# labgem/pangenomeNEM

Measured on AMD Instinct MI355X. Metric: em_family_x_organism_cells_per_sec, higher is better.
Workload: dtype f32 chains with f64 intermediates (reference arithmetic); int32 popcounts in the M-step; 1 GPU; BASELINE configs[1]: 20000 families x 500 organisms, K=3, beta=0.5, contiguity graph (path + 5% chords, weights 1..8), ncem/sk_/pk; U-shaped family-frequency spectrum (Beta(0.3, 0.3) per family), default .m init; families_total=20000, families_per_gpu=20000, organisms=500, K=3, parallelism=1 GPU

## Files before the change

### pangenomenem_amd/csrc/nem_kernels.hip

```cpp
#include <hip/hip_runtime.h>
#include <cstdlib>
#include <algorithm>
#include <cfloat>
#include <cstdint>
#include <cstring>
#include <type_traits>

#include "nem_ff.hpp"
#include "nem_chain.hpp"
#include "nem_halfsum.hpp"
#include "nem_kernels.hpp"
#include "nem_sweep_dev.hpp"

namespace nemk {

#ifdef NEM_PHASE_PROF
__device__ unsigned long long g_phase[32];
#define NEM_PHASE(i) do { if (blockIdx.x == 0 && threadIdx.x == 0) g_phase[i] = wall_clock64(); } while (0)
#else
#define NEM_PHASE(i) do { } while (0)
#endif


__device__ __forceinline__ int stat_sum(const int* __restrict__ stats, int idx, int ranks, int stride)
{
    int s = stats[idx];
    for (int r = 1; r < ranks; r++) s += stats[idx + r * stride];
    return s;
}

__device__ inline int wave_reduce_add(int v)
{
    v += __builtin_amdgcn_update_dpp(0, v, 0xB1, 0xF, 0xF, false);
    v += __builtin_amdgcn_update_dpp(0, v, 0x4E, 0xF, 0xF, false);
    v += __builtin_amdgcn_update_dpp(0, v, 0x141, 0xF, 0xF, false);
    v += __builtin_amdgcn_update_dpp(0, v, 0x140, 0xF, 0xF, false);
    v += __builtin_amdgcn_update_dpp(0, v, 0x142, 0xA, 0xF, false);
    v += __builtin_amdgcn_update_dpp(0, v, 0x143, 0xC, 0xF, false);
    return __builtin_amdgcn_readlane(v, 63);
}

__device__ inline long long wave_reduce_add_ll(long long v)
{
    const int lo = wave_reduce_add((int)(v & 0xFFFFF));
    const int hi = wave_reduce_add((int)(v >> 20));
    return ((long long)hi << 20) + (long long)lo;
}

__device__ __forceinline__ float chain_add16(float s, const float4& a, const float4& b, const float4& c, const float4& d)
{
    asm volatile("v_add_f32 %0, %0, %1\n\tv_add_f32 %0, %0, %2\n\tv_add_f32 %0, %0, %3\n\tv_add_f32 %0, %0, %4\n\t"
                 "v_add_f32 %0, %0, %5\n\tv_add_f32 %0, %0, %6\n\tv_add_f32 %0, %0, %7\n\tv_add_f32 %0, %0, %8\n\t"
                 "v_add_f32 %0, %0, %9\n\tv_add_f32 %0, %0, %10\n\tv_add_f32 %0, %0, %11\n\tv_add_f32 %0, %0, %12\n\t"
// ... 99 lines not shown
    }
}

constexpr int DCH = 512;

__device__ __forceinline__ bool density_tile(int K, int ntiles, int& tile, int& k)
{
    const int b = blockIdx.x;
    const int g = b / (8 * K), r = b - g * (8 * K);
    k = r >> 3;
    tile = g * 8 + (r & 7);
    return tile < ntiles;
}

__device__ __forceinline__ float bern_step(float dk, uint32_t m, int b, double l1h, double l0)
{
    const uint32_t hi = ((b <= 30) ? (m << (30 - b)) : (m >> 1)) & 0x40000000u;
    const double f = __hiloint2double((int)hi, 0);
    return (float)(fma(f, l1h, (double)dk) - l0);
}

__device__ __forceinline__ uint32_t word_of(const uint4& v, int c)
{
    return c == 0 ? v.x : c == 1 ? v.y : c == 2 ? v.z : v.w;
}

__device__ __forceinline__ uint32_t mismatch_word(uint32_t x, const uint2 am)
{
    uint32_t m;
    asm("v_bfi_b32 %0, %1, %2, %3" : "=v"(m) : "v"(x), "v"(am.y), "v"(am.x));
    return m;
}

__device__ __forceinline__ float chain_plain(const uint4* __restrict__ xw4, int npad, int i, int D,
                                    const uint2* am, double l1h, double l0)
{
    float dk = 0.0f;
    const int wlast = (D - 1) >> 5;
    const int glast = wlast >> 2;
    uint4 xn = xw4[i];
    for (int g = 0; g <= glast; g++) {
        const uint4 xv = xn;
        if (g < glast) xn = xw4[(size_t)(g + 1) * npad + i];
#pragma unroll
        for (int c = 0; c < 4; c++) {
            const int w = 4 * g + c;
            if (w > wlast) break;
            const uint32_t m = mismatch_word(word_of(xv, c), am[w]);
            const int nb = (w < wlast) ? 32 : (D - (wlast << 5));
            if (nb == 32) {
#pragma unroll
                for (int b = 0; b < 32; b++) dk = bern_step(dk, m, b, l1h, l0);
            } else {
                for (int b = 0; b < nb; b++) dk = bern_step(dk, m, b, l1h, l0);
            }
        }
    }
    return dk;
}

constexpr int kFFPlainWords = 1;
#ifndef NEM_FF_PLAIN_STEPS
#define NEM_FF_PLAIN_STEPS 32
#endif
constexpr int kFFPlainSteps = NEM_FF_PLAIN_STEPS;

__device__ __forceinline__ void ff_load(const uint32_t* sQ0, const uint32_t* sDQ, uint32_t bits, uint32_t& q0, uint32_t& dq,
                                        uint32_t& end)
{
    const uint32_t E = (bits >> 23) & 255u;
    q0 = sQ0[E];
    dq = sDQ[E];
    end = (E + 1u) << 23;
// ... 48 lines not shown
            bits = ff_probe(mm, j, dq, at);
            bits = ff_exact_step(bits, mm, j, l1h, l0);
            ff_load(sQ0, sDQ, bits, q0, dq, end);
            rem -= (int)j + 1;
            if (rem <= 0) break;
            mm = mm >> (j + 1u);
            const uint32_t c2 = ff_cand(mm, dq, mad24((uint32_t)rem, q0, bits));
            if (c2 < end) { bits = c2; break; }
        }
    }
}

__device__ __forceinline__ void ff_group(const uint4& xv, int g, const uint2* am, uint32_t& bits,
                                         uint32_t& q0, uint32_t& q1, uint32_t& end, const uint32_t* sQ0,
                                         const uint32_t* sQ1, double l1h, double l0)
{
#pragma unroll
    for (int c = 0; c < 4; c++) {
        const int w = 4 * g + c;
        const uint32_t m = mismatch_word(word_of(xv, c), am[w]);
        if (c < kFFPlainWords && g == 0) {
            float dk0 = __uint_as_float(bits);
#pragma unroll
            for (int b = 0; b < kFFPlainSteps; b++) dk0 = bern_step(dk0, m, b, l1h, l0);
            bits = __float_as_uint(dk0);
            ff_load(sQ0, sQ1, bits, q0, q1, end);
            if (kFFPlainSteps < 32) ff_word(bits, q0, q1, end, m >> kFFPlainSteps, 32 - kFFPlainSteps, sQ0, sQ1, l1h, l0);
        } else {
            ff_word(bits, q0, q1, end, m, 32, sQ0, sQ1, l1h, l0);
        }
    }
}

__device__ __forceinline__ float chain_ff(const uint4* __restrict__ xw4, int npad, int i, int D,
                                          const uint2* am, const uint32_t* sQ0,
                                          const uint32_t* sQ1, double l1h, double l0)
{
    const int wlast = (D - 1) >> 5;
    const int gfull = wlast >> 2;
    uint32_t bits = 0u;
    uint32_t q0, q1, end;
    ff_load(sQ0, sQ1, bits, q0, q1, end);
    const uint4* pn = xw4 + i;
    int gi = 0;
    auto next = [&]() {
        const uint4 v = *pn;
        if (gi < gfull) { pn += npad; gi++; }
        return v;
    };
    uint4 x0 = next(), x1 = next(), x2 = next(), x3 = next();
    int g = 0;
    for (; g + 4 <= gfull; g += 4) {
        ff_group(x0, g, am, bits, q0, q1, end, sQ0, sQ1, l1h, l0);
        x0 = next();
        ff_group(x1, g + 1, am, bits, q0, q1, end, sQ0, sQ1, l1h, l0);
        x1 = next();
        ff_group(x2, g + 2, am, bits, q0, q1, end, sQ0, sQ1, l1h, l0);
        x2 = next();
        ff_group(x3, g + 3, am, bits, q0, q1, end, sQ0, sQ1, l1h, l0);
        x3 = next();
    }
    uint4 xt = x0;
    if (g < gfull) { ff_group(x0, g, am, bits, q0, q1, end, sQ0, sQ1, l1h, l0); xt = x1; g++; }
    if (g < gfull) { ff_group(x1, g, am, bits, q0, q1, end, sQ0, sQ1, l1h, l0); xt = x2; g++; }
    if (g < gfull) { ff_group(x2, g, am, bits, q0, q1, end, sQ0, sQ1, l1h, l0); xt = x3; g++; }
#pragma unroll
    for (int c = 0; c < 4; c++) {
        const int w = 4 * gfull + c;
        if (w > wlast) break;
        uint32_t m = mismatch_word(word_of(xt, c), am[w]);
        const int nb = (w < wlast) ? 32 : (D - (wlast << 5));
        if (nb < 32) m &= (1u << nb) - 1u;
        ff_word(bits, q0, q1, end, m, nb, sQ0, sQ1, l1h, l0);
    }
    return __uint_as_float(bits);
}

__device__ __forceinline__ void ff_build(uint32_t* sQ0, uint32_t* sDQ, double l1, double l0, int tid)
{
    uint32_t q0, q1;
    ff_entry(l1, -l0, tid, q0, q1);
    if (q0 == kFFInvalid) q1 = kFFInvalid;
    sQ0[tid] = q0; sDQ[tid] = q1 - q0;
}

__device__ __forceinline__ void density_store(const int* __restrict__ perm, int tile, int tid, int n, int npad, int k,
                                              float dk, uint32_t nul, double pk, float logpk,
                                              double* __restrict__ pkfki, float* __restrict__ logpkfki)
{
    __shared__ double sPk[256];
    __shared__ float sLp[256];
    float logfk; double fk;
    if (!nul) { logfk = -dk; fk = exp((double)logfk); }
    else { logfk = -FLT_MAX; fk = 0.0; }
    const int slot = perm[tile * 256 + tid] - tile * 256;
    sPk[slot] = pk * fk;
    sLp[slot] = logpk + logfk;
    __syncthreads();
    const int io = tile * 256 + tid;
    if (io < n) {
        pkfki[(size_t)k * npad + io] = sPk[tid];
        logpkfki[(size_t)k * npad + io] = sLp[tid];
    }
}

struct DensityArgs {
    const uint4* xw; int n, npad, dpad, D, K;
    const double2* tabT; const double* tabL0; const uint32_t* nz0; const uint32_t* nz1;
    const uint32_t* am0; const uint32_t* am1; const double2* uni; const int* nonuni;
    const double* pk; const float* logpk;
    double* pkfki; float* logpkfki;
    int* zero_flags; int n_zero_flags;
    const int* stop;
    int use_ff;
    const int* perm;
    const uint2* ffq;
};

__device__ __forceinline__ void density_body(const DensityArgs& a)
{
    __shared__ double2 sT[DCH];
    __shared__ double sL[DCH];
    __shared__ uint32_t sQ0[256], sQ1[256];
    __shared__ uint2 sAm[kDensMaskWords];
    if (a.stop != nullptr && *a.stop) return;
    int k, tile;
    if (!density_tile(a.K, a.npad >> 8, tile, k)) return;
    const int tid = threadIdx.x;
    const int i = tile * 256 + tid;
    const int npad = a.npad, dpad = a.dpad;
    const int W = dpad >> 5;
    float dk = 0.0f;
    uint32_t nul = 0;
    if (tile == 0 && k == 0)
        for (int t = tid; t < a.n_zero_flags; t += 256) a.zero_flags[t] = 0;

    if (a.nonuni[k] == 0) {
        const double l1 = a.uni[k].x, l0 = a.uni[k].y;
        const double l1h = 0.5 * l1;
        for (int w = tid; w < W; w += 256) sAm[w] = make_uint2(a.am0[k * W + w], a.am1[k * W + w]);
        if (a.use_ff && l1 >= 0.0 && l0 <= 0.0) {
            const uint2 q = a.ffq[k * 256 + tid];
            sQ0[tid] = q.x; sQ1[tid] = q.y;
            __syncthreads();
            dk = chain_ff(a.xw, npad, i, a.D, sAm, sQ0, sQ1, l1h, l0);
        } else {
            __syncthreads();
            dk = chain_plain(a.xw, npad, i, a.D, sAm, l1h, l0);
        }
    } else {
        for (int d0 = 0; d0 < dpad; d0 += DCH) {
            const int dn = min(DCH, dpad - d0);
            __syncthreads();
            for (int t = tid; t < dn; t += 256) {
                sT[t] = a.tabT[(size_t)k * dpad + d0 + t];
                sL[t] = a.tabL0[(size_t)k * dpad + d0 + t];
            }
            __syncthreads();
            const int w0 = d0 >> 5, wn = dn >> 5;
            const int g0 = w0 >> 2, gn = (wn + 3) >> 2;
            uint4 xnext = a.xw[(size_t)g0 * npad + i];
            for (int g = 0; g < gn; g++) {
                const uint4 xv = xnext;
                if (g + 1 < gn) xnext = a.xw[(size_t)(g0 + g + 1) * npad + i];
#pragma unroll
                for (int c = 0; c < 4; c++) {
                    const int w = 4 * g + c;
                    if (w >= wn) break;
                    const uint32_t x = word_of(xv, c);
                    nul |= (x & a.nz1[k * W + w0 + w]) | (~x & a.nz0[k * W + w0 + w]);
#pragma unroll 8
                    for (int b = 0; b < 32; b++) {
                        const double2 tt = sT[w * 32 + b];
                        const double l0 = sL[w * 32 + b];
                        const double add = ((x >> b) & 1u) ? tt.y : tt.x;
                        dk = (float)(((double)dk + add) - l0);
                    }
                }
            }
        }
    }
    density_store(a.perm, tile, tid, a.n, npad, k, dk, nul, a.pk[k], a.logpk[k], a.pkfki, a.logpkfki);
}

constexpr int FD_MAXD = kFusedMaxD;
constexpr int FD_CH = 256;

struct FusedDensityArgs {
    const uint4* xw; int n, npad, dpad, D, K, n_total, disper, propor;
    const int* stats; int stats_ranks, stats_rank_stride;
    float* center; float* disp; float* prop; float* nbobs_k;
    const float* center_in; const float* disp_in;
    int* iter_flags;
    double* pkfki; float* logpkfki;
    int* zero_flags; int n_zero_flags;
    int* zero_stats; int n_zero_stats;
    const int* stop;
    int use_ff;
    const int* perm;
};

struct StartArgs {
    const float* prop0; const float* center0; const float* disp0;
    int* ctrl; int ctrl_words; int* sweep_next;
};

template <bool START = false>
__device__ __forceinline__ int density_fused_body(const FusedDensityArgs& a, const StartArgs* st = nullptr)
{
    __shared__ __align__(16) float sVal[FD_MAXD];
    __shared__ double2 sT[FD_CH];
    __shared__ double sL[FD_CH];
    __shared__ uint2 sAm[FD_MAXD / 32];
    __shared__ uint32_t sNz0[FD_CH / 32], sNz1[FD_CH / 32];
    __shared__ uint32_t sQ0[256], sQ1[256];
    __shared__ unsigned long long sTot2;
    __shared__ float sEps, sChain[2];
    __shared__ int sGeneral;
    if constexpr (!START) { if (a.stop != nullptr && *a.stop) return -1; }
    int k, tile;
    if (!density_tile(a.K, a.npad >> 8, tile, k)) return -1;
    const int tid = threadIdx.x, lane = tid & 63;
    const int i = tile * 256 + tid;
    const int npad = a.npad, dpad = a.dpad, D = a.D, K = a.K;
    const bool writer = (tile == 0);
    if (tile == 0 && k == 0) {
        for (int t = tid; t < a.n_zero_flags; t += 256) a.zero_flags[t] = 0;
        for (int t = tid; t < a.n_zero_stats; t += 256) a.zero_stats[t] = 0;
        if constexpr (START) {
            for (int t = tid; t < st->ctrl_words; t += 256) if (t != C_FOLD) st->ctrl[t] = 0;
            if (tid == 0) st->sweep_next[0] = 0;
        } else if (tid == 0) {
            int ek = 0;
            for (int c = 0; c < K; c++)
                if (!((double)(float)stat_sum(a.stats, c, a.stats_ranks, a.stats_rank_stride) > kEpsilonD)) ek = c + 1;
            a.iter_flags[FLAG_EMPTYK] = ek;
        }
    }
    if (tid == 0) { sTot2 = 0ull; sGeneral = 0; }
    __syncthreads();

    const int nkI = START ? 0 : stat_sum(a.stats, k, a.stats_ranks, a.stats_rank_stride);
    const float nkf = (float)nkI;
    const bool nonempty = (double)nkf > kEpsilonD;
    long long acc2 = 0;
    int general = 0;
    int differ = 0;
    for (int d = tid; d < dpad; d += 256) {
        float mu = 0.0f, in = 0.0f;
        int a0 = 0, a1 = 0;
        if (d < D) {
            if constexpr (START) {
                mu = st->center0[k * D + d];
                in = st->disp0[k * D + d];
                if (writer) a.disp[k * D + d] = in;
                differ |= (__float_as_uint(in) != __float_as_uint(st->disp0[k * D])) || !((double)in > kEpsilonD);
            } else if (nonempty) {
                const float half = nkf / 2;
                const int s1 = stat_sum(a.stats, K + k * D + d, a.stats_ranks, a.stats_rank_stride);
                const float s0f = (float)(nkI - s1);
                if (s0f > half) { mu = 0.0f; in = (float)s1; }
                else if (s0f == half) { mu = 0.5f; in = 0.5f * nkf; }
                else { mu = 1.0f; in = s0f; }
            } else {
                mu = a.center_in[k * D + d];
            }
            if (writer) a.center[k * D + d] = mu;
            const int ad0 = abs((int)(0.0f - mu)), ad1 = abs((int)(1.0f - mu));
            a0 = (ad0 != 0); a1 = (ad1 != 0);
            if (ad0 > 1 || ad1 > 1) general = 1;
            sVal[d] = in;
            if constexpr (!START) acc2 += (long long)(2.0f * in);
        }
        const uint64_t b0 = __ballot(a0), b1 = __ballot(a1);
        if (lane == 0) {
            const int w = d >> 5;
            sAm[w] = make_uint2((uint32_t)b0, (uint32_t)b1);
            sAm[w + 1] = make_uint2((uint32_t)(b0 >> 32), (uint32_t)(b1 >> 32));
        }
    }
    if constexpr (!START) {
        acc2 = wave_reduce_add_ll(acc2);
        if (lane == 0 && acc2 != 0) atomicAdd(&sTot2, (unsigned long long)acc2);
    }
    if (general) sGeneral = 1;
    bool eps_per_d = false;
    if constexpr (START) eps_per_d = __syncthreads_or(differ) != 0;
    else __syncthreads();

    if constexpr (START) {
        if (tid == 0) sEps = st->disp0[k * D];
    } else if (a.disper == NEMGPU_DISP_K_) {
        if (nkf > 0) {
            const long long cap = 1ll << 24;
            if ((long long)sTot2 <= cap && nkI < (1 << 24)) {
                if (tid == 0) sEps = (0.5f * (float)(long long)sTot2) / ff_repeat_add_u24((uint32_t)nkI, D);
            } else {
                if (tid == 0) {
                    float si = 0.0f;
                    const float4* v4 = reinterpret_cast<const float4*>(sVal);
                    int d = 0;
                    for (; d + 16 <= D; d += 16) si = chain_add16(si, v4[d >> 2], v4[(d >> 2) + 1], v4[(d >> 2) + 2], v4[(d >> 2) + 3]);
                    for (; d < D; d++) si += sVal[d];
                    sChain[0] = si;
                } else if (tid == 64) {
                    if (nkI < (1 << 24)) sChain[1] = ff_repeat_add_u24((uint32_t)nkI, D);
                    else {
                        float sn = 0.0f;
#pragma unroll 8
                        for (int d = 0; d < D; d++) sn += nkf;
                        sChain[1] = sn;
                    }
                }
                __syncthreads();
                if (tid == 0) sEps = sChain[0] / sChain[1];
            }
            __syncthreads();
            const float e = sEps;
            if (writer) for (int d = tid; d < D; d += 256) a.disp[k * D + d] = e;
        } else {
            __syncthreads();
            for (int d = tid; d < D; d += 256) {
                sVal[d] = a.disp_in[k * D + d];
                if (writer) a.disp[k * D + d] = sVal[d];
            }
            eps_per_d = true;
        }
    } else {
        __syncthreads();
        for (int d = tid; d < D; d += 256) {
            float e;
            if (nonempty) e = sVal[d] / nkf;
            else e = a.disp_in[k * D + d];
            if (writer) a.disp[k * D + d] = e;
            sVal[d] = e;
        }
        eps_per_d = true;
    }
    const float propk = START ? st->prop0[k] : (a.propor == NEMGPU_PROP_K) ? nkf / (float)a.n_total : (float)(1.0 / K);
    if (writer && tid == 0) { a.prop[k] = propk; a.nbobs_k[k] = nkf; }
    const double pkd = (double)propk;
    const float logpk = (pkd > kEpsilonD) ? (float)log(pkd) : -INFINITY;
    __syncthreads();

    float dk = 0.0f;
    uint32_t nul = 0;
    const float eps_u = sEps;
    bool uniform = !eps_per_d && !sGeneral && ((double)eps_u > kEpsilonD);
    double l1 = 0.0, l0 = 0.0;
    if (uniform) {
        l1 = log((double)((1.0f - eps_u) / eps_u));
        l0 = log((double)(1.0f - eps_u));
        if (!isfinite(l1) || !isfinite(l0)) uniform = false;
    }
    if (uniform) {
        const double l1h = 0.5 * l1;
        if (a.use_ff && l1 >= 0.0 && l0 <= 0.0) {
            ff_build(sQ0, sQ1, l1, l0, tid);
            __syncthreads();
            dk = chain_ff(a.xw, npad, i, D, sAm, sQ0, sQ1, l1h, l0);
        } else {
            dk = chain_plain(a.xw, npad, i, D, sAm, l1h, l0);
        }
    } else {
        const bool by_mask = nonempty && !sGeneral;
        const float* mu_in = START ? st->center0 : a.center_in;
        for (int d0 = 0; d0 < dpad; d0 += FD_CH) {
            const int dn = min(FD_CH, dpad - d0);
            __syncthreads();
            for (int t = tid; t < dn; t += 256) {
                const int d = d0 + t;
                double t0 = 0.0, t1 = 0.0, ll0 = 0.0;
                int n0 = 0, n1 = 0;
                if (d < D) {
                    const float eps = eps_per_d ? sVal[d] : eps_u;
                    int ad0, ad1;
                    if (nonempty) { ad0 = (sAm[d >> 5].x >> (d & 31)) & 1; ad1 = (sAm[d >> 5].y >> (d & 31)) & 1; }
                    else { const float mu = mu_in[k * D + d]; ad0 = abs((int)(0.0f - mu)); ad1 = abs((int)(1.0f - mu)); }
                    if ((double)eps > kEpsilonD) {
                        const double ll1 = log((double)((1.0f - eps) / eps));
                        ll0 = log((double)(1.0f - eps));
                        t0 = (double)ad0 * ll1;
                        t1 = (double)ad1 * ll1;
                        if (by_mask) { t0 = 0.5 * ll1; t1 = ll0; }
                    } else { n0 = (ad0 != 0); n1 = (ad1 != 0); }
                }
                sT[t] = make_double2(t0, t1);
                sL[t] = ll0;
                const uint64_t m0 = __ballot(n0), m1 = __ballot(n1);
                if (lane == 0) {
                    sNz0[t >> 5] = (uint32_t)m0; sNz0[(t >> 5) + 1] = (uint32_t)(m0 >> 32);
                    sNz1[t >> 5] = (uint32_t)m1; sNz1[(t >> 5) + 1] = (uint32_t)(m1 >> 32);
                }
            }
            __syncthreads();
            const int w0 = d0 >> 5, wn = dn >> 5;
            const int g0 = w0 >> 2, gn = (wn + 3) >> 2;
            uint4 xnext = a.xw[(size_t)g0 * npad + i];
            for (int g = 0; g < gn; g++) {
                const uint4 xv = xnext;
                if (g + 1 < gn) xnext = a.xw[(size_t)(g0 + g + 1) * npad + i];
#pragma unroll
                for (int c = 0; c < 4; c++) {
                    const int w = 4 * g + c;
                    if (w >= wn) break;
                    const uint32_t x = word_of(xv, c);
                    nul |= (x & sNz1[w]) | (~x & sNz0[w]);
                    if (by_mask) {
                        const uint32_t m = mismatch_word(x, sAm[w0 + w]);
#pragma unroll 8
                        for (int b = 0; b < 32; b++) {
                            const double2 cc = sT[w * 32 + b];
                            dk = bern_step(dk, m, b, cc.x, cc.y);
                        }
                    } else {
#pragma unroll 8
                        for (int b = 0; b < 32; b++) {
                            const double2 tt = sT[w * 32 + b];
                            const double c0 = sL[w * 32 + b];
                            const double add = ((x >> b) & 1u) ? tt.y : tt.x;
                            dk = (float)(((double)dk + add) - c0);
                        }
                    }
                }
            }
        }
    }
    density_store(a.perm, tile, tid, a.n, npad, k, dk, nul, pkd, logpk, a.pkfki, a.logpkfki);
    return tile;
}


__device__ __forceinline__ void labels_post_body(int n_local, int lo, int K, int nw64, const uint8_t* __restrict__ lab_new,
                              const uint8_t* __restrict__ lab_old, uint64_t* __restrict__ mask,
                              int* __restrict__ flags, const int* __restrict__ stop, const CtrlArgs& ca, const int nblk)
{
    if (stop != nullptr && *stop) return;
    const int lane = threadIdx.x & 63;
    int any_moved = 0;
    for (int wave = (blockIdx.x * blockDim.x + threadIdx.x) >> 6; wave < nw64; wave += (nblk * blockDim.x) >> 6) {
        const int i = wave * 64 + lane;
        int lab = 255, moved = 0;
        if (i < n_local) {
            lab = lab_new[lo + i] & 0x7F;
            if (lab_old != nullptr) moved = (lab != ((int)lab_old[lo + i] & 0x7F));
        }
        for (int k = 0; k < K; k++) {
            uint64_t m = __ballot(lab == k);
            if (lane == 0) mask[(size_t)k * nw64 + wave] = m;
        }
        any_moved |= __any(moved);
    }
    const int blk_moved = __syncthreads_or(any_moved);
    if (blk_moved && threadIdx.x == 0 && __hip_atomic_load(&flags[FLAG_MOVED], __ATOMIC_RELAXED, __HIP_MEMORY_SCOPE_AGENT) == 0) atomicOr(&flags[FLAG_MOVED], 1);
    if (ca.ctrl != nullptr && last_block_ticket(ca.ticket, nblk)) ctrl_logic(ca);
}

template <int R>
__device__ __forceinline__ void mstep_counts_body(int K, int D, int nw64, const uint64_t* __restrict__ xt,
                                                  const uint64_t* __restrict__ mask, int* __restrict__ stats,
                                                  const int* __restrict__ stop, const CtrlArgs& prev_ctrl, const int bx, const int nblk)
// ... 1457 lines not shown
```

### pangenomenem_amd/csrc/nem_sweep.hip

```cpp
#include <hip/hip_runtime.h>
#include <algorithm>
#include <cstdio>
#include <cstdlib>

#include "nem_kernels.hpp"
#include "nem_sweep_dev.hpp"

namespace nemk {

template <int KT, bool NCEM, int BS, bool LIBC = false, bool COUNT = false>
__global__ __launch_bounds__(BS) void k_sweep(SweepArgs a) { sweep_body<KT, NCEM, BS, LIBC, COUNT>(a, blockIdx.x, gridDim.x); }
template <int KT, bool NCEM, int BS, bool LIBC = false>
__global__ __launch_bounds__(BS) void k_sweep_b(const void* arr, int stride, const int* gx) { NEM_B_HEAD(SweepArgs) sweep_body<KT, NCEM, BS, LIBC>(a, blockIdx.x, nblk); }

static int sweep_variant(int K, bool ncem, bool big, bool libc) { return (K >= 1 && K <= 10 ? K : 0) | (ncem ? 16 : 0) | (big ? 32 : 0) | (libc && ncem ? 64 : 0); }

template <bool BATCHED>
static void sweep_dispatch(int variant, dim3 grid, unsigned bdim, hipStream_t s, const SweepArgs* a, const void* arr, int stride, const int* gx)
{
    const int kt = variant & 15; const bool ncem = (variant & 16) != 0, big = (variant & 32) != 0, libc = (variant & 64) != 0;
    dim3 block(bdim);
#define NEM_SW2(KT_, NC_, BS_, LC_)                                                                                \
    do {                                                                                                           \
        if (BATCHED) hipLaunchKernelGGL((k_sweep_b<KT_, NC_, BS_, LC_>), grid, block, 0, s, arr, stride, gx);     \
// ... 21 lines not shown
    if (big) {
        const int waves_of_blocks = (n_local + 256 * 1024 - 1) / (256 * 1024);
        const int per_block = (n_local + 256 * waves_of_blocks - 1) / (256 * waves_of_blocks);
        bs = std::min(1024, std::max(256, (per_block + 63) / 64 * 64));
    }
    if (big_out) *big_out = big;
    return bs;
}

void launch_sweep(const SweepArgs& a0, bool ncem, hipStream_t s)
{
    bool big = false;
    SweepArgs a = a0;
    const int bs = sweep_block_sites(a.n_local, a.K, &big);
    a.spb = big ? bs : 0;
    dim3 grid((a.n_local + bs - 1) / bs);
    const int variant = sweep_variant(a.K, ncem, big, a.tie_rule == NEMGPU_TIE_LIBC);
    if (a.post_stats != nullptr) {
        if (!(current_recorder() == nullptr && ncem && !big && a.K >= 1 && a.K <= 10 && a.tie_rule != NEMGPU_TIE_LIBC &&
              a.post_on && !a.post_no_masks && a.post_D >= 1 && a.post_D <= kFusedMaxD)) {
            fprintf(stderr, "launch_sweep: no counting round for this shape\n");
            abort();
        }
#define NEM_SWC(KT_) case KT_: hipLaunchKernelGGL((k_sweep<KT_, true, 256, false, true>), grid, dim3(256), 0, s, a); break;
        switch (a.K) { NEM_SWC(1) NEM_SWC(2) NEM_SWC(3) NEM_SWC(4) NEM_SWC(5) NEM_SWC(6) NEM_SWC(7) NEM_SWC(8) NEM_SWC(9) NEM_SWC(10) default: break; }
#undef NEM_SWC
        return;
    }
    if (record_op(OP_SWEEP, variant, grid, (unsigned)bs, a)) return;
    sweep_dispatch<false>(variant, grid, (unsigned)bs, s, &a, nullptr, 0, nullptr);
}


void sweep_dispatch_batched(int variant, dim3 grid, unsigned bdim, hipStream_t s, const void* arr, int stride, const int* gx)
{
    sweep_dispatch<true>(variant, grid, bdim, s, nullptr, arr, stride, gx);
}

}
```

### pangenomenem_amd/csrc/nem_sweep_dev.hpp

```cpp
#pragma once
#include <hip/hip_runtime.h>
#include <cstdint>

#include "nem_kernels.hpp"

namespace nemk {

__host__ __device__ inline uint32_t mix32(uint32_t seed, uint32_t sweep, uint32_t site)
{
    uint32_t h = seed * 0x9E3779B1u + sweep * 0x85EBCA77u + site * 0xC2B2AE3Du + 0x27D4EB2Fu;
    h ^= h >> 16; h *= 0x7FEB352Du;
    h ^= h >> 15; h *= 0x846CA68Bu;
    h ^= h >> 16;
    return h;
}

__device__ inline void ctrl_logic(const CtrlArgs& a)
{
    int* c = a.ctrl;
    constexpr int kMaxRounds = 8;
    const int nr = a.n_rounds > 0 ? (a.n_rounds < kMaxRounds ? a.n_rounds : kMaxRounds) : 2;
    const int stop = c[C_STOP];
    int iters = c[C_ITERS], commits = c[C_COMMITS], sweep_rounds = c[C_SWEEP_ROUNDS], nzero = c[C_NZERO], firstzero = c[C_FIRSTZERO];
    int draws = c[C_DRAWS];
    const int sweep_next = *a.sweep_next;
    const int emptyk = a.iter_flags[FLAG_EMPTYK];
    int moved = __hip_atomic_load(&a.iter_flags[FLAG_MOVED], __ATOMIC_RELAXED, __HIP_MEMORY_SCOPE_AGENT);
    static_assert(FLAG_ROUND_STRIDE == 4 && FLAG_CHANGED == 0 && FLAG_NZERO == 1 && FLAG_FIRSTZERO == 2 && FLAG_NTIES == 3, "a round's slot is one int4");
    int4 rf[kMaxRounds];
#pragma unroll
    for (int r = 0; r < kMaxRounds; r++) rf[r] = r < nr ? reinterpret_cast<const int4*>(a.round0)[r] : make_int4(1, 0, 0, 0);
    int4 bf = make_int4(0, 0, 0, 0);
    bool blind_ok = true;
    int blind_needed = 1;
    if (a.is_init && a.blind != nullptr) {
        if (a.blind_rounds > 1) {
            blind_ok = false;
            for (int q = 0; q < a.blind_rounds && !blind_ok; q++) {
                const int4 f = reinterpret_cast<const int4*>(a.blind)[q];
// ... 174 lines not shown
            for (int k = 0; k < KA; k++) if (k < K) cf[k] = (float)(invz * cinum[k]);
        } else {
            const double invz = 1 / (cum / kEpsilonD);
#pragma unroll
            for (int k = 0; k < KA; k++) if (k < K) cf[k] = (float)(invz * (cinum[k] / kEpsilonD));
        }
        return false;
    }
    const float u = (float)(1.0 / K);
#pragma unroll
    for (int k = 0; k < KA; k++) if (k < K) cf[k] = u;
    return true;
}

constexpr int kLabMask = 0x7F, kLabDrew = 0x80;
constexpr int kTabShort = 1 << 30;
constexpr int kInnerCap = 64;

__device__ __forceinline__ int wave_sum_i32(int v)
{
    v += __builtin_amdgcn_update_dpp(0, v, 0xB1, 0xF, 0xF, false);
    v += __builtin_amdgcn_update_dpp(0, v, 0x4E, 0xF, 0xF, false);
    v += __builtin_amdgcn_update_dpp(0, v, 0x141, 0xF, 0xF, false);
    v += __builtin_amdgcn_update_dpp(0, v, 0x140, 0xF, 0xF, false);
    v += __builtin_amdgcn_update_dpp(0, v, 0x142, 0xA, 0xF, false);
    v += __builtin_amdgcn_update_dpp(0, v, 0x143, 0xC, 0xF, false);
    return __builtin_amdgcn_readlane(v, 63);
}

template <int KT, bool NCEM, int BS, bool LIBC = false, bool COUNT = false>
__device__ __forceinline__ void sweep_body(const SweepArgs& a, const int bx, const int nblk)
{
    static_assert(!COUNT || (NCEM && BS == 256 && !LIBC && KT > 0), "the counting round: NCEM, 256 sites per block");
    int fold_hint = 0;
    if (a.stop != nullptr) {
        static_assert(C_STOP == 0 && C_FOLD == 1, "one 8-byte load");
        const int2 sf = *reinterpret_cast<const int2*>(a.stop);
        if (sf.x) return;
        fold_hint = sf.y;
    }
    bool skip = (a.prev_changed != nullptr && *a.prev_changed == 0);
    if (a.flags_in != nullptr) {
        int any = 0;
        for (int r = 0; r < a.n_ranks; r++) any |= a.flags_in[(size_t)r * a.slot_stride];
        if (!any) skip = true;
    }
    if (skip && !(NCEM && a.post_on)) {
        if (a.publish_byte != nullptr && bx == 0 && threadIdx.x == 0) *a.publish_byte = 0;
        if (LIBC && a.prev_changed != nullptr && bx == 0 && threadIdx.x == 0) a.flags[FLAG_NTIES] = a.prev_changed[FLAG_NTIES - FLAG_CHANGED];
        return;
    }
    __shared__ int s_nzero, s_first;
    __shared__ int s_chg, s_mov;
    constexpr int kExpTab = 64;
    __shared__ double s_exp[NCEM ? kExpTab : 1];
    __shared__ __attribute__((aligned(16))) uint8_t s_lab[NCEM ? BS : 1];
    __shared__ uint64_t s_drew[BS / 64];
    const int spb = (BS > 256 && a.spb > 0) ? a.spb : BS;
    const int i = bx * spb + threadIdx.x;
    const bool active = (int)threadIdx.x < spb && i < a.n_local;
    const int gi = a.lo + (active ? i : 0);
    const int K = KT > 0 ? KT : a.K;
    constexpr int KA = KT > 0 ? KT : kMaxKernelK;
    bool zero_density = false;
    bool changed = false;
    int my_guess = 0, my_old = 0, my_new = 255;
    if (NCEM && active) { my_guess = a.lab_guess[gi]; my_old = a.lab_old[gi] & kLabMask; }
    int blk_cnt_guess = 0;
    if (LIBC && threadIdx.x == 0 && a.tie_cnt_guess != nullptr) blk_cnt_guess = a.tie_cnt_guess[bx];
    constexpr int kCntRows = COUNT ? kFusedMaxD / BS : 1;
    uint64_t xs[kCntRows][4];
    if (COUNT) {
        const int w0 = 4 * bx;
#pragma unroll
        for (int q = 0; q < kCntRows; q++) {
            const int d = (int)threadIdx.x + q * BS;
#pragma unroll
            for (int w = 0; w < 4; w++)
                xs[q][w] = (d < a.post_D && w0 + w < a.post_nw64) ? a.post_xt[(size_t)d * a.post_nw64 + w0 + w] : 0ull;
        }
    }
    __shared__ int s_anydrew;
    if (threadIdx.x == 0) { s_nzero = 0; s_first = 0; s_chg = 0; s_mov = 0; s_anydrew = 0; }
    if (NCEM) s_lab[threadIdx.x] = (uint8_t)my_guess;
    if (NCEM && a.use_nei && !skip && threadIdx.x < kExpTab) s_exp[threadIdx.x] = exp((double)a.beta * (double)(float)threadIdx.x);
    __shared__ int s_lower;
    if (LIBC && !skip && threadIdx.x < 64 && a.tie_cnt_guess != nullptr) {
        int part = 0;
        for (int b = threadIdx.x; b < bx; b += 64) part += a.tie_cnt_guess[b];
        part = wave_sum_i32(part);
        if (threadIdx.x == 0) {
            if (a.rank_tot_in != nullptr)
                for (int r = 0; r < a.rank_index; r++) part += *reinterpret_cast<const int*>(a.rank_tot_in + (size_t)r * a.slot_stride);
            s_lower = part;
        }
    }
    bool blk_drew = false;
    if (LIBC) blk_drew = __syncthreads_or((my_guess & kLabDrew) != 0) != 0;
    else __syncthreads();

    if (NCEM) {
    constexpr bool libc = LIBC;
    const int blk_lo = a.lo + bx * spb;
    double pkf[KA];
#pragma unroll
    for (int k = 0; k < KA; k++) if (k < K) pkf[k] = active && !skip ? a.pkfki[(size_t)k * a.npad + i] : 0.0;
    int nb = 0, ne = 0;
    int dyn[4]; float wn[4]; int fl[4];
#pragma unroll
    for (int u = 0; u < 4; u++) { dyn[u] = -1; wn[u] = 0.0f; fl[u] = 255; }
    if (active && !skip && a.use_nei) {
        nb = a.nei_ptr[i]; ne = a.nei_ptr[i + 1];
        int jn[4];
#pragma unroll
        for (int u = 0; u < 4; u++) {
            const bool ok = nb + u < ne;
            jn[u] = ok ? a.nei_idx[nb + u] : gi;
            wn[u] = ok ? a.nei_w[nb + u] : 0.0f;
        }
#pragma unroll
        for (int u = 0; u < 4; u++) {
            if (nb + u < ne) {
                if (jn[u] < gi && jn[u] >= blk_lo) dyn[u] = jn[u] - blk_lo;
                else fl[u] = ((jn[u] < gi) ? a.lab_guess[jn[u]] : a.lab_old[jn[u]]) & kLabMask;
            }
        }
    }
    const bool long_row = ne - nb > 4;
    int lower_draws = -1;
    bool tab_short = false;
    int cur = my_guess;
    int seen[4] = {-1, -1, -1, -1};
    uint64_t seen_drew = ~0ull; int seen_wave_draws = -1;
    for (int it = 0; it < kInnerCap; it++) {
        int below_in_block = 0;
        uint64_t drew_lt = 0;
        if (libc && blk_drew) {
            const uint64_t bal = __ballot((s_lab[threadIdx.x] & kLabDrew) != 0);
            if ((threadIdx.x & 63) == 0) s_drew[threadIdx.x >> 6] = bal;
            __syncthreads();
            for (int w = 0; w < (int)(threadIdx.x >> 6); w++) below_in_block += (int)__popcll(s_drew[w]);
            drew_lt = s_drew[threadIdx.x >> 6] & ((1ull << (threadIdx.x & 63)) - 1ull);
        }
        int nxt = cur;
        if (active && !skip) {
            int lab[4];
            bool same = it != 0 && !long_row;
#pragma unroll
            for (int u = 0; u < 4; u++) {
                lab[u] = dyn[u] >= 0 ? (s_lab[dyn[u]] & kLabMask) : fl[u];
                same = same && (dyn[u] < 0 || lab[u] == seen[u]);
            }
            if (libc) same = same && drew_lt == seen_drew && below_in_block == seen_wave_draws;
            if (!same) {
                float ctx[KA];
#pragma unroll
                for (int k = 0; k < KA; k++) ctx[k] = 0.0f;
#pragma unroll
                for (int u = 0; u < 4; u++) {
                    seen[u] = lab[u];
                    if (nb + u < ne) {
// ... 79 lines not shown
            if (cnt > 0) atomicAdd(&a.flags[FLAG_NTIES], cnt);
        }
    }
    } else if (active && !skip) {
    float ctx[KA];
    double pkf[KA];
#pragma unroll
    for (int k = 0; k < KA; k++) ctx[k] = 0.0f;
#pragma unroll
    for (int k = 0; k < KA; k++) if (k < K) pkf[k] = a.pkfki[(size_t)k * a.npad + i];
    if (a.use_nei) {
        const int b = a.nei_ptr[i], e = a.nei_ptr[i + 1];
        for (int t = b; t < e; t++) {
            const int j = a.nei_idx[t];
            const float wt = a.nei_w[t];
            const float* row = ((j < gi) ? a.c_guess : a.c_old) + (size_t)j * K;
#pragma unroll
            for (int k = 0; k < KA; k++)
                if (k < K) ctx[k] = ctx[k] + (wt * row[k]);
        }
    }
    float cf[KA];
    zero_density = local_proba<KA>(a, K, pkf, ctx, cf);
    const float* g = a.c_guess + (size_t)gi * K;
    float* o = a.c_out + (size_t)gi * K;
#pragma unroll
    for (int k = 0; k < KA; k++) {
        if (k < K) {
            changed |= (__float_as_uint(cf[k]) != __float_as_uint(g[k]));
            o[k] = cf[k];
        }
    }
    }
    if (__any(changed) && (threadIdx.x & 63) == 0) s_chg = 1;
    int post_lab = 255;
    if (NCEM && a.post_on) {
        int moved = 0;
        if (active) {
            if (skip) post_lab = (a.post_skip_guess ? my_guess : (int)a.lab_out[gi]) & kLabMask;
            else post_lab = a.post_from_guess ? (my_guess & kLabMask) : (my_new != 255 ? my_new : ((int)a.lab_out[gi] & kLabMask));
            if (a.post_moved) moved = (post_lab != my_old);
        }
        if (__any(moved) && (threadIdx.x & 63) == 0) s_mov = 1;
    }
    const uint64_t zmask = __ballot(zero_density);
    if (zmask != 0ull && (threadIdx.x & 63) == 0) {
        atomicAdd(&s_nzero, (int)__popcll(zmask));
        atomicMax(&s_first, a.n_total - (gi + (int)__ffsll((long long)zmask) - 1));
    }
    __syncthreads();
    const bool fold = fold_hint != 0 && a.fold_ticket != nullptr && nblk > 32;
    if (threadIdx.x == 0 && s_nzero > 0) {
        if (!fold) atomicAdd(&a.flags[FLAG_NZERO], s_nzero);
        if (a.flags[FLAG_FIRSTZERO] < s_first) atomicMax(&a.flags[FLAG_FIRSTZERO], s_first);
    }
    if (threadIdx.x == 0) {
        if (s_chg && __hip_atomic_load(&a.flags[FLAG_CHANGED], __ATOMIC_RELAXED, __HIP_MEMORY_SCOPE_AGENT) == 0) atomicOr(&a.flags[FLAG_CHANGED], 1);
        if (NCEM && a.post_on && s_mov && __hip_atomic_load(&a.post_flags[FLAG_MOVED], __ATOMIC_RELAXED, __HIP_MEMORY_SCOPE_AGENT) == 0)
            atomicOr(&a.post_flags[FLAG_MOVED], 1);
    }
    __shared__ uint64_t s_cmask[COUNT ? KA : 1][4];
    if (NCEM && a.post_on) {
        const int wave = i >> 6;
        if (COUNT) {
            for (int k = 0; k < K; k++) {
                const uint64_t m = __ballot(post_lab == k);
// ... 53 lines not shown
```

Baseline: 344.7 billion cells/s.

## Issue entry loads early in fused density and sweep kernels to overlap latency

Moves global loads that sit at kernel entry to the top of the fused density body and the sweep body, before the stop-flag test and barriers. These include the first four xw groups, the perm slot, the per-d stat sums, nk, pkfki, neighbour bounds and labels. The shared-memory atomics for the total and the general flag are replaced with per-wave slots, which removes a zeroing barrier and several __syncthreads around epsilon. The aim is to hide DRAM latency behind the stop check and head barriers. The cost is more registers and loads issued even when the kernel exits early. It also adds optional phase-timing instrumentation and a profiling script.

Result: faster. 353.8 billion cells/s, median of 6 (+2.6%).

```diff
diff --git a/pangenomenem_amd/csrc/nem_kernels.hip b/pangenomenem_amd/csrc/nem_kernels.hip
--- a/pangenomenem_amd/csrc/nem_kernels.hip
+++ b/pangenomenem_amd/csrc/nem_kernels.hip
@@ -17,8 +17,12 @@
 #ifdef NEM_PHASE_PROF
 __device__ unsigned long long g_phase[32];
 #define NEM_PHASE(i) do { if (blockIdx.x == 0 && threadIdx.x == 0) g_phase[i] = wall_clock64(); } while (0)
+#define NEM_PHASE_TAKE(t) const unsigned long long t = wall_clock64()
+#define NEM_PHASE_PUT(i, t) do { if (blockIdx.x == 0 && threadIdx.x == 0) g_phase[i] = t; } while (0)
 #else
 #define NEM_PHASE(i) do { } while (0)
+#define NEM_PHASE_TAKE(t) do { } while (0)
+#define NEM_PHASE_PUT(i, t) do { } while (0)
 #endif
 
 
@@ -184,13 +188,30 @@
     return m;
 }
 
-__device__ __forceinline__ float chain_plain(const uint4* __restrict__ xw4, int npad, int i, int D,
+struct XwHead { uint4 x0, x1, x2, x3; const uint4* pn; int gi; };
+__device__ __forceinline__ uint4 xw_next(const uint4*& pn, int& gi, int gfull, int npad)
+{
+    const uint4 v = *pn;
+    if (gi < gfull) { pn += npad; gi++; }
+    return v;
+}
+__device__ __forceinline__ XwHead xw_head(const uint4* __restrict__ xw4, int npad, int i, int D)
+{
+    const int gfull = ((D - 1) >> 5) >> 2;
+    const uint4* pn = xw4 + i;
+    int gi = 0;
+    const uint4 x0 = xw_next(pn, gi, gfull, npad), x1 = xw_next(pn, gi, gfull, npad);
+    const uint4 x2 = xw_next(pn, gi, gfull, npad), x3 = xw_next(pn, gi, gfull, npad);
+    return XwHead{x0, x1, x2, x3, pn, gi};
+}
+
+__device__ __forceinline__ float chain_plain(const uint4* __restrict__ xw4, const XwHead& h, int npad, int i, int D,
                                     const uint2* am, double l1h, double l0)
 {
     float dk = 0.0f;
     const int wlast = (D - 1) >> 5;
     const int glast = wlast >> 2;
-    uint4 xn = xw4[i];
+    uint4 xn = h.x0;
     for (int g = 0; g <= glast; g++) {
         const uint4 xv = xn;
         if (g < glast) xn = xw4[(size_t)(g + 1) * npad + i];
@@ -305,7 +326,7 @@
     }
 }
 
-__device__ __forceinline__ float chain_ff(const uint4* __restrict__ xw4, int npad, int i, int D,
+__device__ __forceinline__ float chain_ff(const XwHead& h, int npad, int D,
                                           const uint2* am, const uint32_t* sQ0,
                                           const uint32_t* sQ1, double l1h, double l0)
 {
@@ -314,14 +335,10 @@
     uint32_t bits = 0u;
     uint32_t q0, q1, end;
     ff_load(sQ0, sQ1, bits, q0, q1, end);
-    const uint4* pn = xw4 + i;
-    int gi = 0;
-    auto next = [&]() {
-        const uint4 v = *pn;
-        if (gi < gfull) { pn += npad; gi++; }
-        return v;
-    };
-    uint4 x0 = next(), x1 = next(), x2 = next(), x3 = next();
+    const uint4* pn = h.pn;
+    int gi = h.gi;
+    auto next = [&]() { return xw_next(pn, gi, gfull, npad); };
+    uint4 x0 = h.x0, x1 = h.x1, x2 = h.x2, x3 = h.x3;
     int g = 0;
     for (; g + 4 <= gfull; g += 4) {
         ff_group(x0, g, am, bits, q0, q1, end, sQ0, sQ1, l1h, l0);
@@ -357,7 +374,7 @@
     sQ0[tid] = q0; sDQ[tid] = q1 - q0;
 }
 
-__device__ __forceinline__ void density_store(const int* __restrict__ perm, int tile, int tid, int n, int npad, int k,
+__device__ __forceinline__ void density_store(const int* __restrict__ perm, int slot, int tile, int tid, int n, int npad, int k,
                                               float dk, uint32_t nul, double pk, float logpk,
                                               double* __restrict__ pkfki, float* __restrict__ logpkfki)
 {
@@ -366,7 +383,7 @@
     float logfk; double fk;
     if (!nul) { logfk = -dk; fk = exp((double)logfk); }
     else { logfk = -FLT_MAX; fk = 0.0; }
-    const int slot = perm[tile * 256 + tid] - tile * 256;
+    if (perm != nullptr) slot = perm[tile * 256 + tid] - tile * 256;
     sPk[slot] = pk * fk;
     sLp[slot] = logpk + logfk;
     __syncthreads();
@@ -416,10 +433,10 @@
             const uint2 q = a.ffq[k * 256 + tid];
             sQ0[tid] = q.x; sQ1[tid] = q.y;
             __syncthreads();
-            dk = chain_ff(a.xw, npad, i, a.D, sAm, sQ0, sQ1, l1h, l0);
+            dk = chain_ff(xw_head(a.xw, npad, i, a.D), npad, a.D, sAm, sQ0, sQ1, l1h, l0);
         } else {
             __syncthreads();
-            dk = chain_plain(a.xw, npad, i, a.D, sAm, l1h, l0);
+            dk = chain_plain(a.xw, XwHead{a.xw[i]}, npad, i, a.D, sAm, l1h, l0);
         }
     } else {
         for (int d0 = 0; d0 < dpad; d0 += DCH) {
@@ -453,7 +470,7 @@
             }
         }
     }
-    density_store(a.perm, tile, tid, a.n, npad, k, dk, nul, a.pk[k], a.logpk[k], a.pkfki, a.logpkfki);
+    density_store(a.perm, 0, tile, tid, a.n, npad, k, dk, nul, a.pk[k], a.logpk[k], a.pkfki, a.logpkfki);
 }
 
 constexpr int FD_MAXD = kFusedMaxD;
@@ -487,16 +504,45 @@
     __shared__ uint2 sAm[FD_MAXD / 32];
     __shared__ uint32_t sNz0[FD_CH / 32], sNz1[FD_CH / 32];
     __shared__ uint32_t sQ0[256], sQ1[256];
-    __shared__ unsigned long long sTot2;
-    __shared__ float sEps, sChain[2];
-    __shared__ int sGeneral;
-    if constexpr (!START) { if (a.stop != nullptr && *a.stop) return -1; }
+    __shared__ unsigned long long sTot2w[4];
+    __shared__ float sChain[2];
+    __shared__ int sGenW[4];
     int k, tile;
     if (!density_tile(a.K, a.npad >> 8, tile, k)) return -1;
     const int tid = threadIdx.x, lane = tid & 63;
     const int i = tile * 256 + tid;
     const int npad = a.npad, dpad = a.dpad, D = a.D, K = a.K;
     const bool writer = (tile == 0);
+    NEM_PHASE_TAKE(t_entry);
+    XwHead xh{};
+    if constexpr (!START) xh = xw_head(a.xw, npad, i, D);
+    const int slot = a.perm[tile * 256 + tid] - tile * 256;
+    constexpr int kRows = FD_MAXD / 256;
+    int s1w[kRows];
+#pragma unroll
+    for (int q = 0; q < kRows; q++) {
+        s1w[q] = 0;
+        if constexpr (!START) {
+            const int d = tid + 256 * q;
+            if (d < D) s1w[q] = stat_sum(a.stats, K + k * D + d, a.stats_ranks, a.stats_rank_stride);
+        }
+    }
+    int stopw = 0, nkI = 0;
+    if constexpr (!START) {
+        stopw = *(a.stop != nullptr ? a.stop : a.stats);
+        if (a.stop == nullptr) stopw = 0;
+        nkI = stat_sum(a.stats, k, a.stats_ranks, a.stats_rank_stride);
+    }
+    __atomic_signal_fence(__ATOMIC_SEQ_CST);
+    if (stopw) return -1;
+    NEM_PHASE_PUT(16, t_entry);
+    NEM_PHASE(17);
+    const float nkf = (float)nkI;
+    const bool nonempty = (double)nkf > kEpsilonD;
+    const float propk = START ? st->prop0[k] : (a.propor == NEMGPU_PROP_K) ? nkf / (float)a.n_total : (float)(1.0 / K);
+    if (writer && tid == 0) { a.prop[k] = propk; a.nbobs_k[k] = nkf; }
+    const double pkd = (double)propk;
+    const float logpk = (pkd > kEpsilonD) ? (float)log(pkd) : -INFINITY;
     if (tile == 0 && k == 0) {
         for (int t = tid; t < a.n_zero_flags; t += 256) a.zero_flags[t] = 0;
         for (int t = tid; t < a.n_zero_stats; t += 256) a.zero_stats[t] = 0;
@@ -510,16 +556,12 @@
             a.iter_flags[FLAG_EMPTYK] = ek;
         }
     }
-    if (tid == 0) { sTot2 = 0ull; sGeneral = 0; }
-    __syncthreads();
-
-    const int nkI = START ? 0 : stat_sum(a.stats, k, a.stats_ranks, a.stats_rank_stride);
-    const float nkf = (float)nkI;
-    const bool nonempty = (double)nkf > kEpsilonD;
+    NEM_PHASE(18);
+
     long long acc2 = 0;
     int general = 0;
     int differ = 0;
-    for (int d = tid; d < dpad; d += 256) {
+    auto centre_of = [&](const int d, const int s1_d) {
         float mu = 0.0f, in = 0.0f;
         int a0 = 0, a1 = 0;
         if (d < D) {
@@ -530,7 +572,7 @@
                 differ |= (__float_as_uint(in) != __float_as_uint(st->disp0[k * D])) || !((double)in > kEpsilonD);
             } else if (nonempty) {
                 const float half = nkf / 2;
-                const int s1 = stat_sum(a.stats, K + k * D + d, a.stats_ranks, a.stats_rank_stride);
+                const int s1 = s1_d;
                 const float s0f = (float)(nkI - s1);
                 if (s0f > half) { mu = 0.0f; in = (float)s1; }
                 else if (s0f == half) { mu = 0.5f; in = 0.5f * nkf; }
@@ -551,23 +593,32 @@
             sAm[w] = make_uint2((uint32_t)b0, (uint32_t)b1);
             sAm[w + 1] = make_uint2((uint32_t)(b0 >> 32), (uint32_t)(b1 >> 32));
         }
-    }
-    if constexpr (!START) {
-        acc2 = wave_reduce_add_ll(acc2);
-        if (lane == 0 && acc2 != 0) atomicAdd(&sTot2, (unsigned long long)acc2);
-    }
-    if (general) sGeneral = 1;
+    };
+    if constexpr (START) {
+        for (int d = tid; d < dpad; d += 256) centre_of(d, 0);
+    } else {
+#pragma unroll
+        for (int q = 0; q < kRows; q++)
+            if (tid + 256 * q < dpad) centre_of(tid + 256 * q, s1w[q]);
+    }
+    if constexpr (!START) acc2 = wave_reduce_add_ll(acc2);
+    const int gen_w = __any(general);
+    if (lane == 0) { sTot2w[tid >> 6] = (unsigned long long)acc2; sGenW[tid >> 6] = gen_w; }
     bool eps_per_d = false;
     if constexpr (START) eps_per_d = __syncthreads_or(differ) != 0;
     else __syncthreads();
-
+    const long long tot2 = (long long)(sTot2w[0] + sTot2w[1] + sTot2w[2] + sTot2w[3]);
+    const bool any_general = (sGenW[0] | sGenW[1] | sGenW[2] | sGenW[3]) != 0;
+    NEM_PHASE(19);
+
+    float eps_u = 0.0f;
     if constexpr (START) {
-        if (tid == 0) sEps = st->disp0[k * D];
+        eps_u = st->disp0[k * D];
     } else if (a.disper == NEMGPU_DISP_K_) {
         if (nkf > 0) {
             const long long cap = 1ll << 24;
-            if ((long long)sTot2 <= cap && nkI < (1 << 24)) {
-                if (tid == 0) sEps = (0.5f * (float)(long long)sTot2) / ff_repeat_add_u24((uint32_t)nkI, D);
+            if (tot2 <= cap && nkI < (1 << 24)) {
+                eps_u = (0.5f * (float)tot2) / ff_repeat_add_u24((uint32_t)nkI, D);
             } else {
                 if (tid == 0) {
                     float si = 0.0f;
@@ -586,13 +637,10 @@
                     }
                 }
                 __syncthreads();
-                if (tid == 0) sEps = sChain[0] / sChain[1];
-            }
-            __syncthreads();
-            const float e = sEps;
-            if (writer) for (int d = tid; d < D; d += 256) a.disp[k * D + d] = e;
+                eps_u = sChain[0] / sChain[1];
+            }
+            if (writer) for (int d = tid; d < D; d += 256) a.disp[k * D + d] = eps_u;
         } else {
-            __syncthreads();
             for (int d = tid; d < D; d += 256) {
                 sVal[d] = a.disp_in[k * D + d];
                 if (writer) a.disp[k * D + d] = sVal[d];
@@ -600,7 +648,6 @@
             eps_per_d = true;
         }
     } else {
-        __syncthreads();
         for (int d = tid; d < D; d += 256) {
             float e;
             if (nonempty) e = sVal[d] / nkf;
@@ -610,16 +657,11 @@
         }
         eps_per_d = true;
     }
-    const float propk = START ? st->prop0[k] : (a.propor == NEMGPU_PROP_K) ? nkf / (float)a.n_total : (float)(1.0 / K);
-    if (writer && tid == 0) { a.prop[k] = propk; a.nbobs_k[k] = nkf; }
-    const double pkd = (double)propk;
-    const float logpk = (pkd > kEpsilonD) ? (float)log(pkd) : -INFINITY;
-    __syncthreads();
+    NEM_PHASE(20);
 
     float dk = 0.0f;
     uint32_t nul = 0;
-    const float eps_u = sEps;
-    bool uniform = !eps_per_d && !sGeneral && ((double)eps_u > kEpsilonD);
+    bool uniform = !eps_per_d && !any_general && ((double)eps_u > kEpsilonD);
     double l1 = 0.0, l0 = 0.0;
     if (uniform) {
         l1 = log((double)((1.0f - eps_u) / eps_u));
@@ -631,12 +673,16 @@
         if (a.use_ff && l1 >= 0.0 && l0 <= 0.0) {
             ff_build(sQ0, sQ1, l1, l0, tid);
             __syncthreads();
-            dk = chain_ff(a.xw, npad, i, D, sAm, sQ0, sQ1, l1h, l0);
+            NEM_PHASE(21);
+            if constexpr (START) xh = xw_head(a.xw, npad, i, D);
+            dk = chain_ff(xh, npad, D, sAm, sQ0, sQ1, l1h, l0);
         } else {
-            dk = chain_plain(a.xw, npad, i, D, sAm, l1h, l0);
-        }
+            if constexpr (START) xh = xw_head(a.xw, npad, i, D);
+            dk = chain_plain(a.xw, xh, npad, i, D, sAm, l1h, l0);
+        }
+        NEM_PHASE(22);
     } else {
-        const bool by_mask = nonempty && !sGeneral;
+        const bool by_mask = nonempty && !any_general;
         const float* mu_in = START ? st->center0 : a.center_in;
         for (int d0 = 0; d0 < dpad; d0 += FD_CH) {
             const int dn = min(FD_CH, dpad - d0);
@@ -699,7 +745,8 @@
             }
         }
     }
-    density_store(a.perm, tile, tid, a.n, npad, k, dk, nul, pkd, logpk, a.pkfki, a.logpkfki);
+    density_store(nullptr, slot, tile, tid, a.n, npad, k, dk, nul, pkd, logpk, a.pkfki, a.logpkfki);
+    NEM_PHASE(23);
     return tile;
 }
 
diff --git a/pangenomenem_amd/csrc/nem_sweep.hip b/pangenomenem_amd/csrc/nem_sweep.hip
--- a/pangenomenem_amd/csrc/nem_sweep.hip
+++ b/pangenomenem_amd/csrc/nem_sweep.hip
@@ -77,6 +77,13 @@
 }
 
 
+#ifdef NEM_PHASE_PROF
+extern "C" int nemgpu_debug_sweep_phases(unsigned long long* out8)
+{
+    return (int)hipMemcpyFromSymbol(out8, HIP_SYMBOL(g_sweep_phase), sizeof(unsigned long long) * 8);
+}
+#endif
+
 void sweep_dispatch_batched(int variant, dim3 grid, unsigned bdim, hipStream_t s, const void* arr, int stride, const int* gx)
 {
     sweep_dispatch<true>(variant, grid, bdim, s, nullptr, arr, stride, gx);
diff --git a/pangenomenem_amd/csrc/nem_sweep_dev.hpp b/pangenomenem_amd/csrc/nem_sweep_dev.hpp
--- a/pangenomenem_amd/csrc/nem_sweep_dev.hpp
+++ b/pangenomenem_amd/csrc/nem_sweep_dev.hpp
@@ -5,6 +5,17 @@
 #include "nem_kernels.hpp"
 
 namespace nemk {
+
+#ifdef NEM_PHASE_PROF
+static __device__ unsigned long long g_sweep_phase[8];
+#define NEM_SWEEP_PHASE(i) do { if (bx == 0 && threadIdx.x == 0) g_sweep_phase[i] = wall_clock64(); } while (0)
+#define NEM_SWEEP_PHASE_TAKE(t) const unsigned long long t = wall_clock64()
+#define NEM_SWEEP_PHASE_PUT(i, t) do { if (bx == 0 && threadIdx.x == 0) g_sweep_phase[i] = t; } while (0)
+#else
+#define NEM_SWEEP_PHASE(i) do { } while (0)
+#define NEM_SWEEP_PHASE_TAKE(t) do { } while (0)
+#define NEM_SWEEP_PHASE_PUT(i, t) do { } while (0)
+#endif
 
 __host__ __device__ inline uint32_t mix32(uint32_t seed, uint32_t sweep, uint32_t site)
 {
@@ -245,14 +256,58 @@
 __device__ __forceinline__ void sweep_body(const SweepArgs& a, const int bx, const int nblk)
 {
     static_assert(!COUNT || (NCEM && BS == 256 && !LIBC && KT > 0), "the counting round: NCEM, 256 sites per block");
+    static_assert(C_STOP == 0 && C_FOLD == 1, "one 8-byte load");
+    NEM_SWEEP_PHASE_TAKE(t_entry);
+    const int spb = (BS > 256 && a.spb > 0) ? a.spb : BS;
+    const int i = bx * spb + threadIdx.x;
+    const bool active = (int)threadIdx.x < spb && i < a.n_local;
+    const int gi = a.lo + (active ? i : 0);
+    const int K = KT > 0 ? KT : a.K;
+    constexpr int KA = KT > 0 ? KT : kMaxKernelK;
+    int my_guess = 0, my_old = 0, my_new = 255;
+    int blk_cnt_guess = 0;
+    constexpr int kCntRows = COUNT ? kFusedMaxD / BS : 1;
+    uint64_t xs[kCntRows][4];
+    double pkf[NCEM ? KA : 1];
+    int nb = 0, ne = 0;
     int fold_hint = 0;
-    if (a.stop != nullptr) {
-        static_assert(C_STOP == 0 && C_FOLD == 1, "one 8-byte load");
-        const int2 sf = *reinterpret_cast<const int2*>(a.stop);
+    bool skip;
+    if constexpr (NCEM) {
+        if (LIBC && threadIdx.x == 0 && a.tie_cnt_guess != nullptr) blk_cnt_guess = a.tie_cnt_guess[bx];
+        if (COUNT) {
+            const int w0 = 4 * bx;
+#pragma unroll
+            for (int q = 0; q < kCntRows; q++) {
+                const int d = (int)threadIdx.x + q * BS;
+#pragma unroll
+                for (int w = 0; w < 4; w++)
+                    xs[q][w] = (d < a.post_D && w0 + w < a.post_nw64) ? a.post_xt[(size_t)d * a.post_nw64 + w0 + w] : 0ull;
+            }
+        }
+#pragma unroll
+        for (int k = 0; k < KA; k++) if (k < K) pkf[k] = active ? a.pkfki[(size_t)k * a.npad + i] : 0.0;
+        if (active && a.use_nei) { nb = a.nei_ptr[i]; ne = a.nei_ptr[i + 1]; }
+        const int* some = reinterpret_cast<const int*>(a.pkfki);
+        int2 sf = *reinterpret_cast<const int2*>(a.stop != nullptr ? a.stop : some);
+        int pc = *(a.prev_changed != nullptr ? a.prev_changed : some);
+        if (active) { my_guess = a.lab_guess[gi]; my_old = a.lab_old[gi] & kLabMask; }
+        if (a.stop == nullptr) sf = make_int2(0, 0);
+        if (a.prev_changed == nullptr) pc = 1;
+        __atomic_signal_fence(__ATOMIC_SEQ_CST);
+        asm volatile("" :: "s"(pc));
         if (sf.x) return;
         fold_hint = sf.y;
-    }
-    bool skip = (a.prev_changed != nullptr && *a.prev_changed == 0);
+        skip = (pc == 0);
+    } else {
+        if (a.stop != nullptr) {
+            const int2 sf = *reinterpret_cast<const int2*>(a.stop);
+            if (sf.x) return;
+            fold_hint = sf.y;
+        }
+        skip = (a.prev_changed != nullptr && *a.prev_changed == 0);
+    }
+    NEM_SWEEP_PHASE_PUT(0, t_entry);
+    NEM_SWEEP_PHASE(1);
     if (a.flags_in != nullptr) {
         int any = 0;
         for (int r = 0; r < a.n_ranks; r++) any |= a.flags_in[(size_t)r * a.slot_stride];
@@ -269,30 +324,8 @@
     __shared__ double s_exp[NCEM ? kExpTab : 1];
     __shared__ __attribute__((aligned(16))) uint8_t s_lab[NCEM ? BS : 1];
     __shared__ uint64_t s_drew[BS / 64];
-    const int spb = (BS > 256 && a.spb > 0) ? a.spb : BS;
-    const int i = bx * spb + threadIdx.x;
-    const bool active = (int)threadIdx.x < spb && i < a.n_local;
-    const int gi = a.lo + (active ? i : 0);
-    const int K = KT > 0 ? KT : a.K;
-    constexpr int KA = KT > 0 ? KT : kMaxKernelK;
     bool zero_density = false;
     bool changed = false;
-    int my_guess = 0, my_old = 0, my_new = 255;
-    if (NCEM && active) { my_guess = a.lab_guess[gi]; my_old = a.lab_old[gi] & kLabMask; }
-    int blk_cnt_guess = 0;
-    if (LIBC && threadIdx.x == 0 && a.tie_cnt_guess != nullptr) blk_cnt_guess = a.tie_cnt_guess[bx];
-    constexpr int kCntRows = COUNT ? kFusedMaxD / BS : 1;
-    uint64_t xs[kCntRows][4];
-    if (COUNT) {
-        const int w0 = 4 * bx;
-#pragma unroll
-        for (int q = 0; q < kCntRows; q++) {
-            const int d = (int)threadIdx.x + q * BS;
-#pragma unroll
-            for (int w = 0; w < 4; w++)
-                xs[q][w] = (d < a.post_D && w0 + w < a.post_nw64) ? a.post_xt[(size_t)d * a.post_nw64 + w0 + w] : 0ull;
-        }
-    }
     __shared__ int s_anydrew;
     if (threadIdx.x == 0) { s_nzero = 0; s_first = 0; s_chg = 0; s_mov = 0; s_anydrew = 0; }
     if (NCEM) s_lab[threadIdx.x] = (uint8_t)my_guess;
@@ -311,19 +344,15 @@
     bool blk_drew = false;
     if (LIBC) blk_drew = __syncthreads_or((my_guess & kLabDrew) != 0) != 0;
     else __syncthreads();
+    NEM_SWEEP_PHASE(2);
 
     if (NCEM) {
     constexpr bool libc = LIBC;
     const int blk_lo = a.lo + bx * spb;
-    double pkf[KA];
-#pragma unroll
-    for (int k = 0; k < KA; k++) if (k < K) pkf[k] = active && !skip ? a.pkfki[(size_t)k * a.npad + i] : 0.0;
-    int nb = 0, ne = 0;
     int dyn[4]; float wn[4]; int fl[4];
 #pragma unroll
     for (int u = 0; u < 4; u++) { dyn[u] = -1; wn[u] = 0.0f; fl[u] = 255; }
     if (active && !skip && a.use_nei) {
-        nb = a.nei_ptr[i]; ne = a.nei_ptr[i + 1];
         int jn[4];
 #pragma unroll
         for (int u = 0; u < 4; u++) {
@@ -340,6 +369,7 @@
         }
     }
     const bool long_row = ne - nb > 4;
+    NEM_SWEEP_PHASE(3);
     int lower_draws = -1;
     bool tab_short = false;
     int cur = my_guess;
@@ -485,6 +515,7 @@
         }
     }
     }
+    NEM_SWEEP_PHASE(4);
     if (__any(changed) && (threadIdx.x & 63) == 0) s_chg = 1;
     int post_lab = 255;
     if (NCEM && a.post_on) {
diff --git a/profiles/entry_loads_phases.py b/profiles/entry_loads_phases.py
--- /dev/null
+++ b/profiles/entry_loads_phases.py
@@ -0,0 +1,75 @@
+#!/usr/bin/env python3
+import argparse
+import ctypes as C
+import json
+import os
+import statistics
+import sys
+import tempfile
+
+ROOT = os.path.dirname(os.path.dirname(os.path.abspath(__file__)))
+sys.path.insert(0, ROOT)
+
+DENSITY = [(16, "entry (tile known, loads asked for)"), (17, "past the stop test"), (18, "class constants, zeroing loops"),
+           (19, "centres and masks (behind their barrier)"), (20, "epsilon"), (21, "ff tables (behind their barrier)"),
+           (22, "chain"), (23, "stored")]
+SWEEP = [(0, "entry"), (1, "past the stop and previous-round tests"), (2, "head barrier"),
+         (3, "densities, row bounds, first four neighbours"), (4, "block-local steps done, labels stored")]
+
+
+def build_instrumented(where):
+    from pangenomenem_amd import build as b
+    lib = os.path.join(where, "libnem_mi355x.so")
+    if os.path.isfile(lib):
+        return lib
+    b.LIB, b.OBJ = lib, os.path.join(where, "obj")
+    os.environ["NEM_EXTRA_HIPCC_FLAGS"] = (os.environ.get("NEM_EXTRA_HIPCC_FLAGS", "") + " -DNEM_PHASE_PROF").strip()
+    b.build(force=True)
+    return lib
+
+
+def main():
+    ap = argparse.ArgumentParser()
+    ap.add_argument("--dir", default=None)
+    ap.add_argument("--build-only", action="store_true")
+    ap.add_argument("--cycles", type=int, default=20)
+    ap.add_argument("--out", default=None)
+    args = ap.parse_args()
+    where = args.dir or tempfile.mkdtemp(prefix="nem_phase_prof_")
+    os.makedirs(where, exist_ok=True)
+    lib_path = build_instrumented(where)
+    print("instrumented library:", lib_path, file=sys.stderr)
+    if args.build_only:
+        return 0
+    os.environ["NEM_MI355X_LIB"] = lib_path
+    os.environ["NEM_MI355X_GRAPHS"] = "0"
+    import bench
+    from pangenomenem_amd.engine import load_library
+    lib = load_library()
+    lib.nemgpu_debug_phases.argtypes = [C.POINTER(C.c_ulonglong)]
+    lib.nemgpu_debug_sweep_phases.argtypes = [C.POINTER(C.c_ulonglong)]
+    x, nei, prop, center, disp, disper, _ = bench.make_workload(20000, 500, 3, "ushape", 2)
+    run = bench.EngineRun(x, nei, 3, prop, center, disp, "ncem", 0.5, "sk_", tie="hash")
+    run.prime(run.cycle * 4, run.cycle)
+    dens, swp = [], []
+    for _ in range(args.cycles):
+        run.run_steps(run.cycle)
+        d = (C.c_ulonglong * 32)(); s = (C.c_ulonglong * 8)()
+        if lib.nemgpu_debug_phases(d) != 0 or lib.nemgpu_debug_sweep_phases(s) != 0:
+            return 1
+        dens.append([(int(d[i]) - int(d[16])) / 100.0 for i, _ in DENSITY])
+        swp.append([(int(s[i]) - int(s[0])) / 100.0 for i, _ in SWEEP])
+    run.eng.close()
+    out = {"unit": "us since the block's entry, median over %d restart cycles (100 MHz clock: 0.01 us steps)" % args.cycles,
+           "density_fused_body": {name: statistics.median(v[j] for v in dens) for j, (_, name) in enumerate(DENSITY)},
+           "sweep_body": {name: statistics.median(v[j] for v in swp) for j, (_, name) in enumerate(SWEEP)}}
+    text = json.dumps(out, indent=1)
+    print(text)
+    if args.out:
+        with open(args.out, "w") as f:
+            f.write(text + "\n")
+    return 0
+
+
+if __name__ == "__main__":
+    sys.exit(main())
```
